# MichiganCOG/video-frame-inpainting

Measured on AMD Instinct MI355X. Metric: inpainted frames/sec (128x128, K=F=5, T=5), higher is better.
Workload: dtype f32; 1 GPU; configs[1]: bi-TAI (TAI_gray) 128x128 grayscale K=F=5 T=5 inference, batch 32 per GPU, sepconv HIP kernels + hipGraph replay; clips_per_gpu=32, global_clips=32, parallelism=clip-sharded x1, no collective, ranks=1

## Files before the change

### include/tai_sepconv.h

```cpp
#ifndef TAI_SEPCONV_H
#define TAI_SEPCONV_H

#ifdef __cplusplus
extern "C" {
#endif

#define TAI_SEPCONV_OK 0
#define TAI_SEPCONV_EINVAL (-1)
#define TAI_SEPCONV_ELAUNCH (-2)

int tai_sepconv_forward(const float* input, const float* vertical, const float* horizontal,
                        float* output, int B, int C, int H, int W, int ks, void* hip_stream);

int tai_sepconv_backward(const float* grad_output, const float* input, const float* vertical,
                         const float* horizontal, float* grad_input, float* grad_vertical,
                         float* grad_horizontal, int B, int C, int H, int W, int ks,
                         void* hip_stream);

int tai_upsample_bilinear2x_forward(const float* input, float* output, int planes, int H, int W, void* hip_stream);
int tai_upsample_bilinear2x_backward(const float* grad_output, float* grad_input, int planes, int H, int W, void* hip_stream);

int tai_bias_act_inplace(float* x, const float* bias, int N, int C, int HW, int act, void* hip_stream);

int tai_unpool2x_add(const float* x, const float* res, float* out, long long planes, int h, int w, void* hip_stream);

int tai_convlstm_gates_forward(const float* gates, const float* c, float* new_c, float* new_h, int N, int F, int HW,
                               float forget_bias, void* hip_stream);
int tai_convlstm_gates_backward(const float* gates, const float* c, const float* new_c, const float* grad_new_c,
                                const float* grad_new_h, float* grad_gates, float* grad_c, int N, int F, int HW, float forget_bias,
                                void* hip_stream);

int tai_conv_cin1_forward(const float* x, const float* weight, const float* bias, float* y, int N, int Co, int H, int W,
                          int k, int act, void* hip_stream);
int tai_conv_cin1_forward_maxpool(const float* x, const float* weight, const float* bias, float* y, float* ypool, int N, int Co,
                                  int H, int W, int k, int act, void* hip_stream);
int tai_conv_cin1_forward_maxpool_window(const float* x, const float* weight, const float* bias, float* y, float* ypool, int N,
                                         int Co, int H, int W, int k, int act, int pool_h, int pool_w, int pool_oy, int pool_ox,
                                         void* hip_stream);
int tai_conv_cout1_3x3_forward(const float* x, const float* weight, const float* bias, float* y, int N, int Ci, int H,
                               int W, int act, void* hip_stream);
int tai_conv_cout1_5x5_forward(const float* x, const float* weight, const float* bias, float* y, int N, int Ci, int H, int W,
                               void* hip_stream);

int tai_conv_shift_stack(const float* x, float* out, int N, int C, int H, int W, int k, void* hip_stream);

int tai_window_scale_bias_lrelu(float* y, const float* bias, const float* inv_scale, int nw, int B, int C, int HW, float slope,
                                void* hip_stream);
int tai_window_scale_bias_lrelu_scalar(float* y, const float* bias, const float* inv_scale, int nw, int B, int C, int HW, float slope,
                                       void* hip_stream);
int tai_window_scale_lrelu_backward_scalar(const float* grad_y, const float* y, const float* inv_scale, float* grad_z, float* grad_scaled,
                                           int nw, int B, int C, int HW, float slope, void* hip_stream);
int tai_window_scale_lrelu_backward(const float* grad_y, const float* y, const float* inv_scale, float* grad_z, float* grad_scaled,
                                    int nw, int B, int C, int HW, float slope, void* hip_stream);

int tai_thin_conv_wrw(const float* big, const float* thin, float* dw, float* dbias, float* workspace, int N, int Cb, int H, int W,
                      int k, void* hip_stream);

int tai_act_maxpool2x2_forward(const float* z, float* y, float* ypool, long long planes, int H, int W, int relu, void* hip_stream);
int tai_act_maxpool2x2_backward(const float* grad_y, const float* grad_ypool, const float* y, float* grad_z, long long planes, int H,
                                int W, int relu, void* hip_stream);

long long tai_conv3x3_wino_wrw_workspace_floats(int N, int C, int K, int H, int W);
int tai_conv3x3_wino_wrw(const float* x, const float* dy, float* dw, float* dbias, float* workspace, int N, int C, int K, int H,
                         int W, void* hip_stream);
int tai_conv3x3_wino_wrw_window(const float* x, const float* dy, float* dw, float* dbias, float* workspace, int N, int C, int K,
                                int H, int W, int in_h, int in_w, int in_oy, int in_ox, void* hip_stream);
int tai_conv3x3_wino_wrw_set_paired(int on);
int tai_conv3x3_wino_wrw_set_tile(int tile);
int tai_conv3x3_wino_wrw_plan(int N, int C, int K, int H, int W, int in_h, int in_w, int in_oy, int in_ox, int* out);

int tai_sn_power_iteration(float* weight, float* u, float* scratch, float* sigma_out, int out_rows, int in_cols, int Ip,
                           void* hip_stream);

long long tai_conv3x3_wino_weight_floats(int K, int C);
int tai_conv3x3_wino_transform_weights(const float* weight, float* U, int K, int C, void* hip_stream);
int tai_conv3x3_wino_forward(const float* x, const float* U, const float* bias, float* y, int N, int C, int K, int H, int W,
                             int act, void* hip_stream);
int tai_conv3x3_wino_forward_maxpool(const float* x, const float* U, const float* bias, float* y, float* ypool, int N, int C,
                                     int K, int H, int W, int act, void* hip_stream);
int tai_conv3x3_wino_forward_window(const float* x, const float* U, const float* bias, float* y, float* ypool, int N, int C,
                                    int K, int H, int W, int in_h, int in_w, int in_oy, int in_ox, int act, void* hip_stream);
int tai_conv3x3_wino_forward_parts(const float* const* xs, int nparts, const float* U, const float* bias, float* y, int N,
                                   int C, int K, int H, int W, int act, void* hip_stream);
int tai_conv3x3_wino_forward_ex(const float* const* xs, int nparts, int shift_k, const float* U, const float* bias, float* y,
                                float* ypool, int pool_h, int pool_w, int pool_oy, int pool_ox, const float* addx, float* y2, int N,
                                int C, int K, int H, int W, int in_h, int in_w, int in_oy, int in_ox, int act, void* hip_stream);
int tai_conv3x3_wino_forward_plan(int nparts, int shift_k, int has_pool, int has_addx, int has_y2, int N, int C, int K, int H, int W, int in_h,
                                  int in_w, int in_oy, int in_ox, int act, const float* U, int* out);
long long tai_conv3x3_wino43_weight_floats(int K, int C);
int tai_conv3x3_wino43_transform_weights(const float* weight, float* U, int K, int C, void* hip_stream);
int tai_conv3x3_wino43_forward(const float* x, const float* U, const float* bias, float* y, int N, int C, int K, int H, int W, int act,
                               void* hip_stream);
int tai_conv3x3_wino43_forward_ex(const float* const* xs, int nparts, const float* U, const float* bias, float* y, float* ypool,
                                  const float* addx, float* y2, int N, int C, int K, int H, int W, int act, void* hip_stream);
int tai_conv3x3_wino43_forward_blocks(const float* x, int shift_k, const float* U, const float* bias, float* y, float* ypool, int pool_h,
                                      int pool_w, int pool_oy, int pool_ox, int N, int C, int K, int H, int W, int in_h, int in_w, int in_oy,
                                      int in_ox, int act, void* hip_stream);
int tai_conv3x3_wino43_set_waves(int waves);
int tai_conv3x3_wino43_set_placement(int xcd_aware);
int tai_conv3x3_wino43_forward_ws(const float* const* xs, int nparts, const float* U, const float* bias, float* y, float* ypool,
                                  const float* addx, float* y2, float* workspace, long long workspace_floats, int N, int C, int K, int H,
                                  int W, int act, void* hip_stream);
long long tai_conv3x3_wino43_workspace_floats(int N, int C, int K, int H, int W, int nparts);
int tai_conv3x3_wino43_splits(int N, int C, int K, int H, int W, int nparts, int* chunks_per_split);
int tai_conv3x3_wino43_set_splitc(int on);
int tai_conv3x3_wino43_forward_parts(const float* const* xs, int nparts, const float* U, const float* bias, float* y, int N, int C, int K,
                                     int H, int W, int act, void* hip_stream);
int tai_conv3x3_wino_set_arithmetic(int mode);
int tai_conv3x3_wino_get_arithmetic(void);
int tai_conv3x3_wino_forget_weights(const float* U);
int tai_conv3x3_wino_set_tall(int on);
int tai_conv3x3_wino_forward_timeline(const float* x, const float* U, const float* bias, float* y, int N, int C, int K, int H,
                                      int W, long long* stamps, void* hip_stream);
int tai_conv3x3_wino_timeline_skip(int level);

int tai_sepconv_set_forward_variant(int variant);
int tai_sepconv_default_forward_variant(int C, int W, int ks);
int tai_sepconv_forward_route(int B, int C, int H, int W, int ks, int variant);

int tai_sepconv_set_grad_input_variant(int variant);

int tai_sepconv_set_grad_taps_variant(int variant);

long long tai_sepconv_forward_bytes(int B, int C, int H, int W, int ks);
long long tai_sepconv_backward_bytes(int B, int C, int H, int W, int ks);

int tai_hbm_read_probe(const void* buffer, long long bytes, int nt, float* sink, void* hip_stream);

long long tai_conv_bf16_weight_elems(int K, int C, int k);
int tai_conv_bf16_pack_weights(const float* w, void* Wp, int K, int C, int k, int transposed, void* hip_stream);
int tai_conv_bf16_forward(const float* const* xs, int nparts, const void* Wp, const float* bias, float* y, float* ypool,
                          const float* addx, float* y2, int N, int C, int K, int H, int W, int k, int act, void* hip_stream);
int tai_conv_bf16_plan(int N, int K, int H, int W, int k, int* out);

long long tai_frame_metrics_workspace_bytes(int N, int C, int H, int W);
int tai_frame_metrics(const float* pred, const float* gt, long long* sse, double* ssim, double* l2, void* workspace, int N, int C,
                      int H, int W, void* hip_stream);

long long tai_ssim_loss_workspace_bytes(int N, int C, int H, int W);
int tai_ssim_loss(const float* pred, const float* gt, double* plane_ssim, double* totals, float* grad, void* workspace, int N, int C,
                  int H, int W, void* hip_stream);

long long tai_image_loss_workspace_bytes(int npred, long long planes, int H, int W);
int tai_image_loss(const float* const* preds, int npred, const float* gt, int kind, float eps,
                   double* plane_terms , double* totals ,
                   float* const* grads ,
                   void* workspace, long long planes, int H, int W, void* hip_stream);

long long tai_lap_loss_workspace_bytes(long long planes, int H, int W, int levels);
int tai_lap_loss(const float* pred, const float* gt, int levels, double* plane_terms ,
                 double* totals , float* grad ,
                 void* workspace, long long planes, int H, int W, void* hip_stream);

long long tai_temporal_loss_workspace_bytes(int npred, int B, int T, int C, int H, int W);
int tai_temporal_loss(const float* const* preds, int npred, const float* gt,
                      const long long* strides ,
                      int kind, float eps,
                      double* seq_terms , double* totals ,
                      float* const* grads ,
                      void* workspace, int B, int T, int C, int H, int W, void* stream );

long long tai_census_loss_workspace_bytes(int npred, int B, int T, int C, int H, int W);
int tai_census_loss(const float* const* preds, int npred, const float* gt,
                    const long long* strides ,
                    double* frame_terms , double* totals ,
                    float* const* grads ,
                    void* workspace, int B, int T, int C, int H, int W, void* stream );

int tai_clip_from_frames(const unsigned char* frames, long long frames_bytes, const long long* table, const long long* table_host,
                         const float* levels, float* out, int N, int c_dim, int H, int W, int pad_h, int pad_w, void* hip_stream);
int tai_frames_to_uint8(const float* x, unsigned char* out, int N, int C, int Hs, int Ws, int h, int w, int reverse_channels,
                        void* hip_stream);

int tai_clip_from_frames_aug(const unsigned char* frames, long long frames_bytes, const long long* table, const long long* table_host,
                             const float* tables, int n_tables, const float* levels, float* out, int N, int c_dim, int H, int W, int pad_h,
                             int pad_w, void* stream );

long long tai_state_digest_workspace_bytes(int n_entries, long long n_segments);
int tai_state_digest(const long long* table, const long long* table_host, int n_entries, long long n_segments, long long seg_words,
                     void* workspace, unsigned long long* result, void* hip_stream);

long long tai_grad_stats_workspace_bytes(int n_entries, long long n_segments);
int tai_grad_stats(const long long* table, const long long* table_host, int n_entries, long long n_segments, int blocks, void* workspace,
                   double* sumsq, float* maxabs, long long* nonfinite, void* hip_stream);
long long tai_grad_scale_workspace_bytes(int n_entries, long long n_segments);
int tai_grad_scale(const long long* table, const long long* table_host, int n_entries, long long n_segments, float c, int blocks,
                   void* workspace, void* hip_stream);

long long tai_step_verdict_workspace_bytes(void);
int tai_step_verdict(const double* sumsq, const long long* nonfinite, int n_entries, double max_norm, int which, int close_update,
                     long long patience, long long table_len, long long* record, void* hip_stream);
long long tai_fused_step_workspace_bytes(int n_entries, long long n_segments);
int tai_fused_step(const long long* table, const long long* table_host, int n_entries, long long n_segments, const float* scalars,
                   long long table_len, float w1, float b2, float w2, float eps, float wE, const long long* record, int which, int nt,
                   int blocks, void* workspace, void* hip_stream);

const char* tai_sepconv_last_error(void);

int tai_sepconv_version(void);

const char* tai_sepconv_source_hash(void);

#ifdef __cplusplus
}
#endif
#endif
```

### video-frame-inpainting_amd/csrc/capi_pointwise.inc

```

extern "C" {

int tai_hbm_read_probe(const void* buffer, long long bytes, int nt, float* sink, void* hip_stream) {
    g_err[0] = 0;
    if (!buffer || !sink || bytes < (1 << 20)) return fail(TAI_SEPCONV_EINVAL, "%s", "hbm_read_probe: needs a buffer of at least 1 MiB and a sink of 4096 floats");
    hipStream_t s = static_cast<hipStream_t>(hip_stream);
    const size_t n4 = (size_t)bytes / 16;
    hipLaunchKernelGGL(nt ? probe::stream_read<true> : probe::stream_read<false>, dim3(4096), dim3(256), 0, s,
                       static_cast<const probe::f4v*>(buffer), sink, n4);
    return check_launch("hbm_read_probe");
}

int tai_bias_act_inplace(float* x, const float* bias, int N, int C, int HW, int act, void* hip_stream) {
    g_err[0] = 0;
    if (!x || !bias) return fail(TAI_SEPCONV_EINVAL, "%s", "null pointer");
    if (N <= 0 || C <= 0 || HW <= 0 || act < 0 || act > 2) return fail(TAI_SEPCONV_EINVAL, "%s", "bad dimensions or activation");
    hipStream_t s = static_cast<hipStream_t>(hip_stream);
    const long long n = (long long)N * C * HW;
    const bool vec = (HW % 4 == 0) && ((reinterpret_cast<uintptr_t>(x) & 15) == 0);
    const long long work = vec ? n / 4 : n;
    const int blocks = grid_for(work, 16384);
    if (vec) {
        auto kern = act == bact::ACT_RELU ? bact::bias_act_vec4<bact::ACT_RELU>
                  : act == bact::ACT_TANH ? bact::bias_act_vec4<bact::ACT_TANH> : bact::bias_act_vec4<bact::ACT_NONE>;
        hipLaunchKernelGGL(kern, dim3(blocks), dim3(256), 0, s, x, bias, n / 4, HW / 4, C);
    } else {
        auto kern = act == bact::ACT_RELU ? bact::bias_act_scalar<bact::ACT_RELU>
                  : act == bact::ACT_TANH ? bact::bias_act_scalar<bact::ACT_TANH> : bact::bias_act_scalar<bact::ACT_NONE>;
        hipLaunchKernelGGL(kern, dim3(blocks), dim3(256), 0, s, x, bias, n, HW, C);
    }
    return check_launch("bias_act");
}

int tai_conv_cin1_forward(const float* x, const float* weight, const float* bias, float* y, int N, int Co, int H, int W,
                          int k, int act, void* hip_stream) {
    g_err[0] = 0;
    if (!x || !weight || !bias || !y) return fail(TAI_SEPCONV_EINVAL, "%s", "null pointer");
    if (N <= 0 || Co <= 0 || H <= 0 || W <= 0 || W % 4 != 0 || (k != 3 && k != 5) || act < 0 || act > 1)
        return fail(TAI_SEPCONV_EINVAL, "%s", "conv_cin1: needs W % 4 == 0, k in {3, 5}, act in {0, 1}");
    hipStream_t s = static_cast<hipStream_t>(hip_stream);
    const long long work = (long long)N * H * (W / 4);
    const int blocks = grid_for(work, 8192);
    const int cgroups = (work < 4 * 262144 && Co >= 16) ? 4 : 1;
    auto kern = k == 3 ? (act == 0 ? thin::conv_cin1<3, 0> : thin::conv_cin1<3, 1>) : (act == 0 ? thin::conv_cin1<5, 0> : thin::conv_cin1<5, 1>);
    hipLaunchKernelGGL(kern, dim3(blocks, cgroups), dim3(256), 0, s, x, weight, bias, y, N, Co, H, W);
    return check_launch("conv_cin1");
}

int tai_conv_cin1_forward_maxpool_window(const float* x, const float* weight, const float* bias, float* y, float* ypool, int N,
                                         int Co, int H, int W, int k, int act, int pool_h, int pool_w, int pool_oy, int pool_ox,
                                         void* hip_stream) {
    g_err[0] = 0;
    if (!x || !weight || !bias || !y || !ypool) return fail(TAI_SEPCONV_EINVAL, "%s", "null pointer");
    if (N <= 0 || Co <= 0 || H <= 0 || W <= 0 || W % 4 != 0 || H % 2 != 0 || (k != 3 && k != 5) || act < 0 || act > 1)
        return fail(TAI_SEPCONV_EINVAL, "%s", "conv_cin1_maxpool: needs W % 4 == 0, even H, k in {3, 5}, act in {0, 1}");
    if (pool_oy < 0 || pool_ox < 0 || pool_h < H / 2 + pool_oy || pool_w < W / 2 + pool_ox)
        return fail(TAI_SEPCONV_EINVAL, "%s", "conv_cin1_maxpool: bad pooled-output window");
    hipStream_t s = static_cast<hipStream_t>(hip_stream);
    const long long work = (long long)N * (H / 2) * (W / 4);
    const int blocks = grid_for(work, 8192);
    const int cgroups = (work < 4 * 262144 && Co >= 16) ? 4 : 1;
    auto kern = k == 3 ? (act == 0 ? thin::conv_cin1_pool<3, 0> : thin::conv_cin1_pool<3, 1>)
                       : (act == 0 ? thin::conv_cin1_pool<5, 0> : thin::conv_cin1_pool<5, 1>);
    hipLaunchKernelGGL(kern, dim3(blocks, cgroups), dim3(256), 0, s, x, weight, bias, y, ypool, N, Co, H, W, pool_h, pool_w, pool_oy, pool_ox);
    return check_launch("conv_cin1_maxpool");
}

int tai_conv_cin1_forward_maxpool(const float* x, const float* weight, const float* bias, float* y, float* ypool, int N, int Co,
                                  int H, int W, int k, int act, void* hip_stream) {
    return tai_conv_cin1_forward_maxpool_window(x, weight, bias, y, ypool, N, Co, H, W, k, act, H / 2, W / 2, 0, 0, hip_stream);
}

int tai_unpool2x_add(const float* x, const float* res, float* out, long long planes, int h, int w, void* hip_stream) {
    g_err[0] = 0;
    if (!x || !res || !out) return fail(TAI_SEPCONV_EINVAL, "%s", "null pointer");
    if (planes <= 0 || h <= 0 || w <= 0 || w % 2 != 0) return fail(TAI_SEPCONV_EINVAL, "%s", "unpool2x_add: needs even w");
    const long long work = planes * 2 * h * (2 * w / 4);
    const int blocks = grid_for(work, 16384);
    hipLaunchKernelGGL(bact::unpool2x_add, dim3(blocks), dim3(256), 0, static_cast<hipStream_t>(hip_stream), x, res, out, planes, h, w);
    return check_launch("unpool2x_add");
}

int tai_convlstm_gates_forward(const float* gates, const float* c, float* new_c, float* new_h, int N, int F, int HW,
                               float forget_bias, void* hip_stream) {
    g_err[0] = 0;
    if (!gates || !c || !new_c || !new_h) return fail(TAI_SEPCONV_EINVAL, "%s", "null pointer");
    if (N <= 0 || F <= 0 || HW <= 0 || HW % 4 != 0) return fail(TAI_SEPCONV_EINVAL, "%s", "convlstm_gates: needs HW % 4 == 0");
    const long long work = (long long)N * F * (HW / 4);
    const int blocks = grid_for(work, 16384);
    hipLaunchKernelGGL(bact::convlstm_gates, dim3(blocks), dim3(256), 0, static_cast<hipStream_t>(hip_stream), gates, c, new_c,
                       new_h, N, F, HW / 4, forget_bias);
    return check_launch("convlstm_gates");
}

int tai_sn_power_iteration(float* weight, float* u, float* scratch, float* sigma_out, int out_rows, int in_cols, int Ip,
                           void* hip_stream) {
    g_err[0] = 0;
    if (!weight || !u || !scratch) return fail(TAI_SEPCONV_EINVAL, "%s", "null pointer");
    if (out_rows <= 0 || in_cols <= 0 || Ip <= 0 || Ip > 64) return fail(TAI_SEPCONV_EINVAL, "%s", "sn_power_iteration: bad shape or Ip");
    hipStream_t stream = static_cast<hipStream_t>(hip_stream);
    float* v_raw = scratch;
    float* t_raw = scratch + in_cols;
    float* sigma = sigma_out;
    const dim3 wt_block(snorm::WT_COLS, snorm::WT_ROWGROUPS);
    const int wt_grid = (in_cols + snorm::WT_COLS - 1) / snorm::WT_COLS;
    for (int it = 0; it < Ip; ++it) {
        hipLaunchKernelGGL(snorm::wt_u, dim3(wt_grid), wt_block, 0, stream, weight, it == 0 ? u : t_raw, v_raw, out_rows, in_cols,
                           it == 0 ? 0 : 1);
        hipLaunchKernelGGL(snorm::w_v, dim3(out_rows), dim3(256), 0, stream, weight, v_raw, t_raw, in_cols);
    }
    const long long n = (long long)out_rows * in_cols;
    const long long want = (n / 4 + 255) / 256;
    const int blocks = (int)(want < 1 ? 1 : (want > 1024 ? 1024 : want));
    hipLaunchKernelGGL(snorm::finish, dim3(blocks), dim3(256), 0, stream, weight, t_raw, u, sigma, out_rows, n);
    return check_launch("sn_power_iteration");
}

int tai_window_scale_bias_lrelu(float* y, const float* bias, const float* inv_scale, int nw, int B, int C, int HW, float slope,
                                void* hip_stream) {
    g_err[0] = 0;
    if (!y || !bias || !inv_scale) return fail(TAI_SEPCONV_EINVAL, "%s", "null pointer");
    if (nw <= 0 || B <= 0 || C <= 0 || HW <= 0 || HW % 4 != 0) return fail(TAI_SEPCONV_EINVAL, "%s", "window_scale_bias_lrelu: needs HW % 4 == 0");
    const long long n4 = (long long)nw * B * C * (HW / 4);
    const int blocks = grid_for(n4, 16384);
    hipLaunchKernelGGL(snorm::window_scale_bias_lrelu, dim3(blocks), dim3(256), 0, static_cast<hipStream_t>(hip_stream), y, bias,
                       inv_scale, n4, C * (HW / 4), HW / 4, C, B, slope);
    return check_launch("window_scale_bias_lrelu");
}

int tai_window_scale_lrelu_backward(const float* grad_y, const float* y, const float* inv_scale, float* grad_z, float* grad_scaled,
                                    int nw, int B, int C, int HW, float slope, void* hip_stream) {
    g_err[0] = 0;
    if (!grad_y || !y || !inv_scale || !grad_z || !grad_scaled) return fail(TAI_SEPCONV_EINVAL, "%s", "null pointer");
    if (nw <= 0 || B <= 0 || C <= 0 || HW <= 0 || HW % 4 != 0) return fail(TAI_SEPCONV_EINVAL, "%s", "window_scale_lrelu_backward: needs HW % 4 == 0");
    const long long n4 = (long long)nw * B * C * (HW / 4);
    const int blocks = grid_for(n4, 16384);
    hipLaunchKernelGGL(snorm::window_scale_lrelu_backward, dim3(blocks), dim3(256), 0, static_cast<hipStream_t>(hip_stream), grad_y, y,
                       inv_scale, grad_z, grad_scaled, n4, C * (HW / 4), B, slope);
    return check_launch("window_scale_lrelu_backward");
}

int tai_window_scale_bias_lrelu_scalar(float* y, const float* bias, const float* inv_scale, int nw, int B, int C, int HW, float slope,
                                       void* hip_stream) {
    g_err[0] = 0;
    if (!y || !bias || !inv_scale) return fail(TAI_SEPCONV_EINVAL, "%s", "null pointer");
    if (nw <= 0 || B <= 0 || C <= 0 || HW <= 0 || (long long)nw * B * C >= (1LL << 31))
        return fail(TAI_SEPCONV_EINVAL, "%s", "window_scale_bias_lrelu_scalar: bad dimensions");
    const int planes = nw * B * C;
    const int blocks = planes < 16384 ? planes : 16384;
    hipLaunchKernelGGL(snorm::window_scale_bias_lrelu_scalar, dim3(blocks), dim3(256), 0, static_cast<hipStream_t>(hip_stream), y, bias,
                       inv_scale, planes, HW, C, B, slope);
    return check_launch("window_scale_bias_lrelu_scalar");
}

int tai_window_scale_lrelu_backward_scalar(const float* grad_y, const float* y, const float* inv_scale, float* grad_z, float* grad_scaled,
                                           int nw, int B, int C, int HW, float slope, void* hip_stream) {
    g_err[0] = 0;
    if (!grad_y || !y || !inv_scale || !grad_z || !grad_scaled) return fail(TAI_SEPCONV_EINVAL, "%s", "null pointer");
    if (nw <= 0 || B <= 0 || C <= 0 || HW <= 0 || (long long)nw * B * C >= (1LL << 31))
        return fail(TAI_SEPCONV_EINVAL, "%s", "window_scale_lrelu_backward_scalar: bad dimensions");
    const int planes = nw * B * C;
    const int blocks = planes < 16384 ? planes : 16384;
    hipLaunchKernelGGL(snorm::window_scale_lrelu_backward_scalar, dim3(blocks), dim3(256), 0, static_cast<hipStream_t>(hip_stream), grad_y,
                       y, inv_scale, grad_z, grad_scaled, planes, HW, C, B, slope);
    return check_launch("window_scale_lrelu_backward_scalar");
}

int tai_thin_conv_wrw(const float* big, const float* thin, float* dw, float* dbias, float* workspace, int N, int Cb, int H, int W,
                      int k, void* hip_stream) {
    g_err[0] = 0;
    if (!big || !thin || !workspace || (!dw && !dbias)) return fail(TAI_SEPCONV_EINVAL, "%s", "null pointer");
    if (N <= 0 || Cb <= 0 || H <= 0 || W <= 0 || W % 4 != 0 || (k != 3 && k != 5) || (long long)N * Cb > 0x7fffffffLL)
        return fail(TAI_SEPCONV_EINVAL, "%s", "thin_conv_wrw: needs W % 4 == 0 and k in {3, 5}");
    hipStream_t stream = static_cast<hipStream_t>(hip_stream);
    hipLaunchKernelGGL(k == 3 ? thin::thin_wrw<3> : thin::thin_wrw<5>, dim3(N * Cb), dim3(256), 0, stream, big, thin, workspace, N, Cb, H, W);
    if (int rc = check_launch("thin_conv_wrw")) return rc;
    const int total = Cb * (k * k + 1);
    hipLaunchKernelGGL(thin::thin_wrw_reduce, dim3((total + 255) / 256), dim3(256), 0, stream, workspace, dw, dbias, N, Cb, k * k);
    return check_launch("thin_conv_wrw_reduce");
}

int tai_act_maxpool2x2_forward(const float* z, float* y, float* ypool, long long planes, int H, int W, int relu, void* hip_stream) {
    g_err[0] = 0;
    if (!z || !y || !ypool) return fail(TAI_SEPCONV_EINVAL, "%s", "null pointer");
    if (planes <= 0 || H <= 0 || W <= 0 || H % 2 != 0 || W % 4 != 0) return fail(TAI_SEPCONV_EINVAL, "%s", "act_maxpool2x2: needs even H and W % 4 == 0");
    const long long work = planes * (H / 2) * (W / 4);
    const int blocks = grid_for(work, 16384);
    hipLaunchKernelGGL(bact::act_pool2x2_forward, dim3(blocks), dim3(256), 0, static_cast<hipStream_t>(hip_stream), z, y, ypool, planes,
                       H, W, relu ? 1 : 0);
    return check_launch("act_maxpool2x2_forward");
}

int tai_act_maxpool2x2_backward(const float* grad_y, const float* grad_ypool, const float* y, float* grad_z, long long planes, int H,
                                int W, int relu, void* hip_stream) {
    g_err[0] = 0;
    if (!y || !grad_z) return fail(TAI_SEPCONV_EINVAL, "%s", "null pointer");
    if (planes <= 0 || H <= 0 || W <= 0 || H % 2 != 0 || W % 4 != 0) return fail(TAI_SEPCONV_EINVAL, "%s", "act_maxpool2x2: needs even H and W % 4 == 0");
    const long long work = planes * (H / 2) * (W / 4);
    const int blocks = grid_for(work, 16384);
    hipLaunchKernelGGL(bact::act_pool2x2_backward, dim3(blocks), dim3(256), 0, static_cast<hipStream_t>(hip_stream), grad_y, grad_ypool,
                       y, grad_z, planes, H, W, relu ? 1 : 0);
    return check_launch("act_maxpool2x2_backward");
}

int tai_convlstm_gates_backward(const float* gates, const float* c, const float* new_c, const float* grad_new_c,
                                const float* grad_new_h, float* grad_gates, float* grad_c, int N, int F, int HW, float forget_bias,
                                void* hip_stream) {
    g_err[0] = 0;
    if (!gates || !c || !new_c || !grad_gates || !grad_c || (!grad_new_c && !grad_new_h)) return fail(TAI_SEPCONV_EINVAL, "%s", "null pointer");
    if (N <= 0 || F <= 0 || HW <= 0 || HW % 4 != 0) return fail(TAI_SEPCONV_EINVAL, "%s", "convlstm_gates: needs HW % 4 == 0");
    const long long work = (long long)N * F * (HW / 4);
    const int blocks = grid_for(work, 16384);
    hipLaunchKernelGGL(bact::convlstm_gates_backward, dim3(blocks), dim3(256), 0, static_cast<hipStream_t>(hip_stream), gates, c,
                       new_c, grad_new_c, grad_new_h, grad_gates, grad_c, N, F, HW / 4, forget_bias);
    return check_launch("convlstm_gates_backward");
}

int tai_conv_shift_stack(const float* x, float* out, int N, int C, int H, int W, int k, void* hip_stream) {
    g_err[0] = 0;
    if (!x || !out) return fail(TAI_SEPCONV_EINVAL, "%s", "null pointer");
    if (N <= 0 || C <= 0 || H <= 0 || W <= 0 || W % 4 != 0 || (k != 5 && k != 7))
        return fail(TAI_SEPCONV_EINVAL, "%s", "conv_shift_stack: needs W % 4 == 0 and k in {5, 7}");
    const int S = k == 5 ? 2 : 3;
    const long long work = (long long)N * S * S * C * (H + 2) * ((W + 4) / 4);
    const int blocks = grid_for(work, 16384);
    hipLaunchKernelGGL(thin::shift_stack, dim3(blocks), dim3(256), 0, static_cast<hipStream_t>(hip_stream), x, out, N, C, H, W, S, k);
    return check_launch("conv_shift_stack");
}

int tai_conv_cout1_3x3_forward(const float* x, const float* weight, const float* bias, float* y, int N, int Ci, int H,
                               int W, int act, void* hip_stream) {
    g_err[0] = 0;
    if (!x || !weight || !bias || !y) return fail(TAI_SEPCONV_EINVAL, "%s", "null pointer");
    if (N <= 0 || Ci <= 0 || H <= 0 || W <= 0 || W % 4 != 0 || act < 0 || act > 2)
        return fail(TAI_SEPCONV_EINVAL, "%s", "conv_cout1: needs W % 4 == 0, act in {0, 1, 2}");
    hipStream_t s = static_cast<hipStream_t>(hip_stream);
    const long long work = (long long)N * H * (W / 4);
    const int blocks = grid_for(work, 8192);
    auto kern = act == 0 ? thin::conv_cout1_3x3<0> : act == 1 ? thin::conv_cout1_3x3<1> : thin::conv_cout1_3x3<2>;
    hipLaunchKernelGGL(kern, dim3(blocks), dim3(256), 0, s, x, weight, bias, y, N, Ci, H, W);
    return check_launch("conv_cout1_3x3");
}

int tai_conv_cout1_5x5_forward(const float* x, const float* weight, const float* bias, float* y, int N, int Ci, int H, int W,
                               void* hip_stream) {
    g_err[0] = 0;
    if (!x || !weight || !y) return fail(TAI_SEPCONV_EINVAL, "%s", "null pointer");
    if (N <= 0 || Ci <= 0 || H <= 0 || W <= 0 || W % 4 != 0) return fail(TAI_SEPCONV_EINVAL, "%s", "conv_cout1_5x5: needs W % 4 == 0");
    const long long work = (long long)N * H * (W / 4);
    const int blocks = grid_for(work, 8192);
    hipLaunchKernelGGL(thin::conv_cout1_5x5, dim3(blocks), dim3(256), 0, static_cast<hipStream_t>(hip_stream), x, weight, bias, y, N, Ci,
                       H, W);
    return check_launch("conv_cout1_5x5");
}

int tai_upsample_bilinear2x_backward(const float* grad_output, float* grad_input, int planes, int H, int W, void* hip_stream) {
    g_err[0] = 0;
    if (!grad_output || !grad_input) return fail(TAI_SEPCONV_EINVAL, "%s", "null pointer");
    if (planes <= 0 || H <= 0 || W <= 0) return fail(TAI_SEPCONV_EINVAL, "%s", "bad dimensions");
    const float rh = (2 * H > 1) ? (float)(H - 1) / (float)(2 * H - 1) : 0.f;
    const float rw = (2 * W > 1) ? (float)(W - 1) / (float)(2 * W - 1) : 0.f;
    const long long work = (long long)planes * H * ((W + 3) / 4);
    const int blocks = grid_for(work, 65536);
    hipLaunchKernelGGL(ups::upsample2x_align_corners_backward, dim3(blocks), dim3(256), 0, static_cast<hipStream_t>(hip_stream),
                       grad_output, grad_input, planes, H, W, rh, rw);
    return check_launch("upsample_bilinear2x_backward");
}

int tai_upsample_bilinear2x_forward(const float* input, float* output, int planes, int H, int W, void* hip_stream) {
    g_err[0] = 0;
    if (!input || !output) return fail(TAI_SEPCONV_EINVAL, "%s", "null pointer");
    if (planes <= 0 || H <= 0 || W <= 0) return fail(TAI_SEPCONV_EINVAL, "%s", "bad dimensions");
    hipStream_t s = static_cast<hipStream_t>(hip_stream);
    const float rh = (2 * H > 1) ? (float)(H - 1) / (float)(2 * H - 1) : 0.f;
    const float rw = (2 * W > 1) ? (float)(W - 1) / (float)(2 * W - 1) : 0.f;
    const long long total = (long long)planes * 2 * H * (2 * W);
    if ((2 * W) % 4 == 0 && H >= 2 && W >= 2 && (long long)H * W * 4 < (1LL << 30)) {
        const int per_plane = H * (2 * W / 4);
        const int bx = grid_for(per_plane, 64);
        hipLaunchKernelGGL(ups::upsample2x_align_corners_pairs, dim3(bx, planes < 65535 ? planes : 65535), dim3(256), 0, s, input, output, planes, H, W,
                           rh, rw);
    } else if ((2 * W) % 4 == 0) {
        const long long threads = total / 4;
        const int blocks = grid_for(threads, 65536);
        hipLaunchKernelGGL(ups::upsample2x_align_corners_quads, dim3(blocks), dim3(256), 0, s, input, output, planes, H,
                           W, rh, rw);
    } else {
        const int blocks = grid_for(total, 65536);
        hipLaunchKernelGGL(ups::upsample2x_align_corners_scalar, dim3(blocks), dim3(256), 0, s, input, output, planes,
                           H, W, rh, rw);
    }
    return check_launch("upsample2x_align_corners");
}

}
```

### video-frame-inpainting_amd/csrc/sepconv_capi.hip

```cpp
#include <hip/hip_runtime.h>

#include <atomic>
#include <cmath>
#include <cstdint>
#include <cstdio>
#include <cstring>
#include <mutex>
#include <unordered_set>

#include "tai_sepconv.h"

#include "sepconv_fwd.hip.inc"
#include "sepconv_bwd.hip.inc"
#include "upsample.hip.inc"
#include "bias_act.hip.inc"
#include "thin_conv.hip.inc"
#include "wino_conv.hip.inc"
#include "wino_split.hip.inc"
#include "wino43_conv.hip.inc"
#include "wino_wrw.hip.inc"
#include "conv_bf16.hip.inc"
#include "spectral_norm.hip.inc"
#include "hbm_probe.hip.inc"
#include "frame_metrics.hip.inc"
#include "ssim_loss.hip.inc"
#include "image_loss.hip.inc"
#include "lap_loss.hip.inc"
#include "temporal_loss.hip.inc"
#include "census_loss.hip.inc"
#include "clip_pipeline.hip.inc"
#include "clip_augment.hip.inc"
#include "state_digest.hip.inc"
#include "grad_stats.hip.inc"
#include "fused_step.hip.inc"

namespace {

thread_local char g_err[256] = "";

int fail(int code, const char* fmt, const char* what) {
    std::snprintf(g_err, sizeof(g_err), fmt, what);
    return code;
}

int check_launch(const char* what) {
    const hipError_t e = hipGetLastError();
    if (e != hipSuccess) {
        std::snprintf(g_err, sizeof(g_err), "%s: %s", what, hipGetErrorString(e));
        return TAI_SEPCONV_ELAUNCH;
    }
    return TAI_SEPCONV_OK;
}

template <typename KernelT>
int allow_lds(KernelT kernel, size_t bytes) {
    if (bytes <= 64 * 1024) return TAI_SEPCONV_OK;
    constexpr int SLOTS = 64;
    static thread_local const void* done_kernel[SLOTS];
    static thread_local size_t done_bytes[SLOTS];
    static thread_local int done_device[SLOTS];
    static thread_local int n_done = 0;
    int device = -1;
    if (hipGetDevice(&device) != hipSuccess) return fail(TAI_SEPCONV_ELAUNCH, "%s", "hipGetDevice");
    const void* key = reinterpret_cast<const void*>(kernel);
    for (int i = 0; i < n_done; ++i)
        if (done_kernel[i] == key && done_device[i] == device && done_bytes[i] >= bytes) return TAI_SEPCONV_OK;
    const hipError_t e = hipFuncSetAttribute(key, hipFuncAttributeMaxDynamicSharedMemorySize, (int)bytes);
    if (e != hipSuccess) {
        std::snprintf(g_err, sizeof(g_err), "hipFuncSetAttribute(lds=%zu): %s", bytes, hipGetErrorString(e));
        return TAI_SEPCONV_ELAUNCH;
    }
    if (n_done < SLOTS) { done_kernel[n_done] = key; done_bytes[n_done] = bytes; done_device[n_done] = device; ++n_done; }
    return TAI_SEPCONV_OK;
}

static int device_cu_count() {
    static thread_local int cached_device = -1, cached_cus = 0;
    int device = -1;
    if (hipGetDevice(&device) != hipSuccess) return 0;
    if (device != cached_device) {
        int n = 0;
        if (hipDeviceGetAttribute(&n, hipDeviceAttributeMultiprocessorCount, device) != hipSuccess) return 0;
        cached_device = device; cached_cus = n;
    }
    return cached_cus;
}

template <typename... P, typename... A>
int launch(void (*kern)(P...), dim3 grid, dim3 block, size_t lds, hipStream_t s, A... args) {
    if (int rc = allow_lds(kern, lds)) return rc;
    hipLaunchKernelGGL(kern, grid, block, lds, s, static_cast<P>(args)...);
    return TAI_SEPCONV_OK;
}

int grid_for(long long work, int cap) {
    const long long blocks = (work + 255) / 256;
    return (int)(blocks < cap ? blocks : cap);
}

bool aligned(const void* p, uintptr_t bytes) { return reinterpret_cast<uintptr_t>(p) % bytes == 0; }

size_t rowloop_lds(int rows, int waves, size_t extra = 0) {
    const size_t patch = (size_t)(rows + 50) * 180 * sizeof(float);
    return ((patch + 1023) & ~(size_t)1023) + (size_t)waves * TAI_FWD_ROWLOOP_RING_SLOTS * 1024 + extra;
}

void wino_div_magic(long long d, unsigned& m, unsigned& sh) {
    if (d <= 1) { m = 0; sh = 0; return; }
    int lg = 0;
    while ((2LL << lg) <= d) ++lg;
    if ((1LL << lg) == d) --lg;
    sh = (unsigned)lg;
    const unsigned __int128 num = (unsigned __int128)1 << (32 + lg);
    m = (unsigned)((num + (unsigned __int128)d - 1) / (unsigned __int128)d);
}

}

extern "C" {

int tai_sepconv_version(void) { return 860; }

const char* tai_sepconv_last_error(void) { return g_err; }

#ifndef TAI_SOURCE_HASH
#define TAI_SOURCE_HASH "unknown"
#endif
static const char k_source_hash[] = "TAI_SOURCE_HASH=" TAI_SOURCE_HASH;
const char* tai_sepconv_source_hash(void) { return k_source_hash + 16; }

}

#include "capi_sepconv.inc"
#include "capi_pointwise.inc"
#include "capi_wino43.inc"
#include "capi_wino.inc"
#include "capi_bf16.inc"
#include "capi_image.inc"
#include "capi_tables.inc"
```

Baseline: 3498 frames/s.

## Add row-strip register-blocked kernels for cout1 3x3 conv and bilinear upsample

Adds a 3x3 single-output-channel conv kernel in which each thread computes a strip of rows by 4 columns. It double-buffers input-channel groups in registers and gets horizontal neighbours with DPP lane shifts instead of redundant loads. It also adds a 2x align-corners upsample kernel that walks many output rows per block, reusing the loaded input rows in a sliding window. Both are enabled by default through a runtime toggle and are meant to cut redundant global loads and launch overhead, at the cost of more register pressure and extra complexity at the edges.

```diff
diff --git a/include/tai_sepconv.h b/include/tai_sepconv.h
--- a/include/tai_sepconv.h
+++ b/include/tai_sepconv.h
@@ -39,6 +39,7 @@
                                          void* hip_stream);
 int tai_conv_cout1_3x3_forward(const float* x, const float* weight, const float* bias, float* y, int N, int Ci, int H,
                                int W, int act, void* hip_stream);
+int tai_stream_fwd_set(int on);
 int tai_conv_cout1_5x5_forward(const float* x, const float* weight, const float* bias, float* y, int N, int Ci, int H, int W,
                                void* hip_stream);
 
diff --git a/video-frame-inpainting_amd/csrc/capi_pointwise.inc b/video-frame-inpainting_amd/csrc/capi_pointwise.inc
--- a/video-frame-inpainting_amd/csrc/capi_pointwise.inc
+++ b/video-frame-inpainting_amd/csrc/capi_pointwise.inc
@@ -228,6 +228,9 @@
     return check_launch("conv_shift_stack");
 }
 
+static std::atomic<int> g_stream_fwd{1};
+int tai_stream_fwd_set(int on) { return g_stream_fwd.exchange(on ? 1 : 0, std::memory_order_relaxed); }
+
 int tai_conv_cout1_3x3_forward(const float* x, const float* weight, const float* bias, float* y, int N, int Ci, int H,
                                int W, int act, void* hip_stream) {
     g_err[0] = 0;
@@ -235,6 +238,15 @@
     if (N <= 0 || Ci <= 0 || H <= 0 || W <= 0 || W % 4 != 0 || act < 0 || act > 2)
         return fail(TAI_SEPCONV_EINVAL, "%s", "conv_cout1: needs W % 4 == 0, act in {0, 1, 2}");
     hipStream_t s = static_cast<hipStream_t>(hip_stream);
+    constexpr int SR = sfw::CONV_ROWS, SU = sfw::CONV_CHANNELS;
+    const int strips = (H + SR - 1) / SR;
+    const long long strip_groups = ((long long)N * strips * (W / 4) + 255) / 256;
+    if (g_stream_fwd.load(std::memory_order_relaxed) && strip_groups <= 0x7fffffffLL) {
+        auto rows = act == 0 ? sfw::conv_cout1_3x3_rows<0, SR, SU, false, false>
+                  : act == 1 ? sfw::conv_cout1_3x3_rows<1, SR, SU, false, false> : sfw::conv_cout1_3x3_rows<2, SR, SU, false, false>;
+        hipLaunchKernelGGL(rows, dim3((unsigned)strip_groups), dim3(256), 0, s, x, weight, bias, y, N, Ci, H, W, strips);
+        return check_launch("conv_cout1_3x3_rows");
+    }
     const long long work = (long long)N * H * (W / 4);
     const int blocks = grid_for(work, 8192);
     auto kern = act == 0 ? thin::conv_cout1_3x3<0> : act == 1 ? thin::conv_cout1_3x3<1> : thin::conv_cout1_3x3<2>;
@@ -275,6 +287,14 @@
     const float rh = (2 * H > 1) ? (float)(H - 1) / (float)(2 * H - 1) : 0.f;
     const float rw = (2 * W > 1) ? (float)(W - 1) / (float)(2 * W - 1) : 0.f;
     const long long total = (long long)planes * 2 * H * (2 * W);
+    if (g_stream_fwd.load(std::memory_order_relaxed) && (2 * W) % 4 == 0 && H >= 2 && W >= 2 && 2 * W / 4 <= sfw::UPS_MAX_QUADS &&
+        (long long)H * W * 4 < (1LL << 30)) {
+        const int side = 256 / (2 * W / 4);
+        const int groups = (planes + side - 1) / side;
+        hipLaunchKernelGGL((sfw::upsample2x_align_corners_rows<sfw::UPS_ROWS, true>), dim3((2 * H + sfw::UPS_ROWS - 1) / sfw::UPS_ROWS, groups < 65535 ? groups : 65535),
+                           dim3(256), 0, s, input, output, planes, H, W, rh, rw);
+        return check_launch("upsample2x_align_corners");
+    }
     if ((2 * W) % 4 == 0 && H >= 2 && W >= 2 && (long long)H * W * 4 < (1LL << 30)) {
         const int per_plane = H * (2 * W / 4);
         const int bx = grid_for(per_plane, 64);
diff --git a/video-frame-inpainting_amd/csrc/sepconv_capi.hip b/video-frame-inpainting_amd/csrc/sepconv_capi.hip
--- a/video-frame-inpainting_amd/csrc/sepconv_capi.hip
+++ b/video-frame-inpainting_amd/csrc/sepconv_capi.hip
@@ -15,6 +15,7 @@
 #include "upsample.hip.inc"
 #include "bias_act.hip.inc"
 #include "thin_conv.hip.inc"
+#include "stream_fwd.hip.inc"
 #include "wino_conv.hip.inc"
 #include "wino_split.hip.inc"
 #include "wino43_conv.hip.inc"
diff --git a/video-frame-inpainting_amd/csrc/stream_fwd.hip.inc b/video-frame-inpainting_amd/csrc/stream_fwd.hip.inc
--- /dev/null
+++ b/video-frame-inpainting_amd/csrc/stream_fwd.hip.inc
@@ -0,0 +1,186 @@
+
+namespace sfw {
+
+typedef float f4v __attribute__((ext_vector_type(4)));
+
+constexpr int CONV_ROWS = 2;
+constexpr int CONV_CHANNELS = 4;
+constexpr int UPS_ROWS = 32;
+constexpr int UPS_MAX_QUADS = 256;
+
+template <bool NT>
+__device__ __forceinline__ f4v load16(const float* p) {
+    const f4v* q = reinterpret_cast<const f4v*>(p);
+    return NT ? __builtin_nontemporal_load(q) : *q;
+}
+
+template <bool NT>
+__device__ __forceinline__ void store16(float* p, f4v v) {
+    f4v* q = reinterpret_cast<f4v*>(p);
+    if (NT) __builtin_nontemporal_store(v, q);
+    else *q = v;
+}
+
+template <int R>
+struct StripRows {
+    f4v m[R + 2];
+    float l[R + 2], r[R + 2];
+};
+
+template <int ACT, int R, int U, bool NT, bool REV>
+__global__ __launch_bounds__(256)
+void conv_cout1_3x3_rows(const float* __restrict__ x, const float* __restrict__ w, const float* __restrict__ bias,
+                         float* __restrict__ y, int N, int Ci, int H, int W, int strips) {
+    const int qw = W / 4;
+    const long long total = (long long)N * strips * qw;
+    const long long idx = (long long)blockIdx.x * 256 + threadIdx.x;
+    if (idx >= total) return;
+    const int q = (int)(idx % qw);
+    const int s = (int)((idx / qw) % strips);
+    const int nn = (int)(idx / ((long long)qw * strips));
+    const int n = REV ? N - 1 - nn : nn;
+    const int x0 = 4 * q, y0 = s * R;
+    const int rows = min(R, H - y0);
+    long long off[R + 2];
+#pragma unroll
+    for (int j = 0; j < R + 2; ++j) off[j] = (long long)min(max(y0 - 1 + j, 0), H - 1) * W + x0;
+    const bool topz = y0 == 0;
+    const int botj = H - 1 - y0;
+    const bool hasl = x0 > 0, hasr = x0 + 4 < W;
+    const int lane = threadIdx.x & 63;
+    const bool own_l = hasl && lane == 0, own_r = hasr && lane == 63;
+    const float* img = x + (long long)n * Ci * H * W;
+    const long long plane_sz = (long long)H * W;
+
+    const float b = bias[0];
+    float a[R][4];
+#pragma unroll
+    for (int j = 0; j < R; ++j) a[j][0] = a[j][1] = a[j][2] = a[j][3] = b;
+
+    auto load_group = [&](int c0, StripRows<R>* buf) {
+#pragma unroll
+        for (int u = 0; u < U; ++u) {
+            const float* plane = img + (long long)min(c0 + u, Ci - 1) * plane_sz;
+#pragma unroll
+            for (int j = 0; j < R + 2; ++j) {
+                buf[u].m[j] = load16<NT>(plane + off[j]);
+                buf[u].l[j] = own_l ? plane[off[j] - 1] : 0.f;
+                buf[u].r[j] = own_r ? plane[off[j] + 4] : 0.f;
+            }
+        }
+    };
+    auto use_group = [&](int c0, StripRows<R>* buf) {
+#pragma unroll
+        for (int u = 0; u < U; ++u) {
+            const int ci = c0 + u;
+            if (ci < Ci) {
+                float L[R + 2], Rr[R + 2];
+#pragma unroll
+                for (int j = 0; j < R + 2; ++j) {
+                    const float fl = __int_as_float(__builtin_amdgcn_update_dpp(0, __float_as_int(buf[u].m[j].w), 0x138, 0xf, 0xf, false));
+                    const float fr = __int_as_float(__builtin_amdgcn_update_dpp(0, __float_as_int(buf[u].m[j].x), 0x130, 0xf, 0xf, false));
+                    L[j] = hasl ? (own_l ? buf[u].l[j] : fl + 0.f) : 0.f;
+                    Rr[j] = hasr ? (own_r ? buf[u].r[j] : fr + 0.f) : 0.f;
+                }
+                float wv[3][3];
+#pragma unroll
+                for (int t = 0; t < 9; ++t) wv[t / 3][t % 3] = w[ci * 9 + t];
+#pragma unroll
+                for (int jj = 0; jj < R; ++jj) {
+#pragma unroll
+                    for (int r = 0; r < 3; ++r) {
+                        const bool zero = (r == 0 && jj == 0 && topz) || (r == 2 && jj == botj);
+                        const float w0 = zero ? 0.f : wv[r][0], w1 = zero ? 0.f : wv[r][1], w2 = zero ? 0.f : wv[r][2];
+                        const f4v m = buf[u].m[jj + r];
+                        a[jj][0] = fmaf(w0, L[jj + r], fmaf(w1, m.x, fmaf(w2, m.y, a[jj][0])));
+                        a[jj][1] = fmaf(w0, m.x, fmaf(w1, m.y, fmaf(w2, m.z, a[jj][1])));
+                        a[jj][2] = fmaf(w0, m.y, fmaf(w1, m.z, fmaf(w2, m.w, a[jj][2])));
+                        a[jj][3] = fmaf(w0, m.z, fmaf(w1, m.w, fmaf(w2, Rr[jj + r], a[jj][3])));
+                    }
+                }
+            }
+        }
+    };
+
+    StripRows<R> bufa[U], bufb[U];
+    load_group(0, bufa);
+    for (int c0 = 0; c0 < Ci; c0 += 2 * U) {
+        if (c0 + U < Ci) load_group(c0 + U, bufb);
+        use_group(c0, bufa);
+        if (c0 + 2 * U < Ci) load_group(c0 + 2 * U, bufa);
+        if (c0 + U < Ci) use_group(c0 + U, bufb);
+    }
+
+    float* out = y + ((long long)n * H + y0) * W + x0;
+#pragma unroll
+    for (int jj = 0; jj < R; ++jj) {
+        if (jj < rows) {
+            f4v v = {a[jj][0], a[jj][1], a[jj][2], a[jj][3]};
+            if (ACT == 1) { v.x = fmaxf(v.x, 0.f); v.y = fmaxf(v.y, 0.f); v.z = fmaxf(v.z, 0.f); v.w = fmaxf(v.w, 0.f); }
+            if (ACT == 2) { v.x = tanhf(v.x); v.y = tanhf(v.y); v.z = tanhf(v.z); v.w = tanhf(v.w); }
+            store16<false>(out + (long long)jj * W, v);
+        }
+    }
+}
+
+template <int K, bool NT>
+__global__ __launch_bounds__(256)
+void upsample2x_align_corners_rows(const float* __restrict__ in, float* __restrict__ out, int planes, int H, int W,
+                                   float rh, float rw) {
+    const int OW = 2 * W, OH = 2 * H, QW = OW / 4;
+    const int P = 256 / QW;
+    const int psub = threadIdx.x / QW, q = threadIdx.x - psub * QW;
+    if (psub >= P) return;
+    unsigned ca[4], cb[4];
+    float w0[4], w1[4];
+#pragma unroll
+    for (int i = 0; i < 4; ++i) {
+        float sx = __fmul_rn(rw, (float)(4 * q + i));
+        asm("" : "+v"(sx));
+        const int x1 = (int)sx;
+        const int xp = (x1 < W - 1) ? 1 : 0;
+        w1[i] = sx - x1; w0[i] = 1.f - w1[i];
+        ca[i] = (unsigned)(psub * H * W + x1); cb[i] = ca[i] + xp;
+    }
+    const unsigned oq = (unsigned)(psub * 4 * H * W + 4 * q);
+    const int oy0 = blockIdx.x * K, oy_end = min(oy0 + K, OH);
+    for (int g = blockIdx.y; g * P < planes; g += gridDim.y) {
+        if (g * P + psub >= planes) return;
+        const float* src = in + (long long)g * P * H * W;
+        float* dst = out + (long long)g * P * 4 * H * W;
+        auto row_of = [&](int oy, float& h0, float& h1) {
+            const float sy = __int_as_float(__builtin_amdgcn_readfirstlane(__float_as_int(__fmul_rn(rh, (float)oy))));
+            const int y1 = (int)sy;
+            h1 = sy - y1; h0 = 1.f - h1;
+            return y1;
+        };
+        float top[8], bot[8], nxt[8];
+        auto load_row = [&](int yrow, float* t) {
+            const float* rp = src + (long long)min(yrow, H - 1) * W;
+#pragma unroll
+            for (int i = 0; i < 4; ++i) { t[i] = rp[ca[i]]; t[4 + i] = rp[cb[i]]; }
+        };
+        float h0, h1;
+        int ycur = row_of(oy0, h0, h1);
+        load_row(ycur, top);
+        load_row(ycur + 1, bot);
+        load_row(ycur + 2, nxt);
+        for (int oy = oy0; oy < oy_end; ++oy) {
+            const int y1 = row_of(oy, h0, h1);
+            if (y1 != ycur) {
+#pragma unroll
+                for (int i = 0; i < 8; ++i) { top[i] = bot[i]; bot[i] = nxt[i]; }
+                ycur = y1;
+                load_row(ycur + 2, nxt);
+            }
+            f4v v;
+            v.x = ups::lerp4(top[0], top[4], bot[0], bot[4], w0[0], w1[0], h0, h1);
+            v.y = ups::lerp4(top[1], top[5], bot[1], bot[5], w0[1], w1[1], h0, h1);
+            v.z = ups::lerp4(top[2], top[6], bot[2], bot[6], w0[2], w1[2], h0, h1);
+            v.w = ups::lerp4(top[3], top[7], bot[3], bot[7], w0[3], w1[3], h0, h1);
+            store16<NT>(dst + (long long)oy * OW + oq, v);
+        }
+    }
+}
+
+}
```

Result: no change. 3516 frames/s (median of 6 runs) (+0.5%).
